# Accustomer/CUDA-AKAZE

Hardware: AMD Instinct MI355X
Metric: pairs_per_sec_detect_describe_match_1080p (higher is better)
Workload: dtype f32; 1 GPU; configs[1]: 1920x1080 grayscale pairs, 4 octaves x 4 sublevels, PM_G2, MLDB-486, max_pts 10000, float path; detect+describe both images + match, D2H included; pairs_per_launch_sequence=256, distinct_pairs_per_gpu=16, float_sequences_enqueued=77, octave_streams=one stream per context, step_pipeline=2, rank0_gpu_numa_node=0

## Files before the change

cuda-akaze_amd/akaze_hip/__init__.py:

```python
import ctypes as C
import os

import numpy as np

try:
    import torch as _torch
except ImportError:
    _torch = None

_HERE = os.path.dirname(os.path.abspath(__file__))
LIB_PATH = os.environ.get("HAK_LIB") or os.path.join(os.path.dirname(_HERE), "libhipakaze.so")

FLEN = 61
MAX_DIST = 96
PM_G1, PM_G2, WEICKERT, CHARBONNIER = 0, 1, 2, 3

POINT_DTYPE = np.dtype([
    ("x", "<f4"), ("y", "<f4"), ("octave", "<i4"), ("response", "<f4"), ("size", "<f4"), ("angle", "<f4"),
    ("features", "u1", (FLEN,)), ("_pad", "u1", (3,)),
    ("match", "<i4"), ("distance", "<i4"), ("match_x", "<f4"), ("match_y", "<f4"),
])
assert POINT_DTYPE.itemsize == 104
MATCH_PAIR_DTYPE = np.dtype([("query", "<i4"), ("train", "<i4"), ("distance", "<i4"), ("second", "<i4"),
                             ("x1", "<f4"), ("y1", "<f4"), ("x2", "<f4"), ("y2", "<f4")])
# ... 100 lines not shown
    "hak_op_hessian": (C.c_int, [_vp, _vp, _vp, _vp, C.c_int, C.c_int, C.c_int, C.c_int]),
    "hak_op_fast_conv_u8": (C.c_int, [_vp, C.c_int, _vp, C.c_int, C.c_int, C.c_int, C.c_float, C.c_int]),
    "hak_op_fast_lowpass": (C.c_int, [_vp, _vp, C.c_int, C.c_int, C.c_int, C.c_float, C.c_int]),
    "hak_op_fast_base": (C.c_int, [_vp, C.c_int, _vp, C.c_int, C.c_int, C.c_int, C.c_float, C.c_int, C.c_float, _ip, _ip, _ip, _ip]),
    "hak_op_fast_down_smooth": (C.c_int, [_vp, _vp, _vp, C.c_int, C.c_int, C.c_int, C.c_int, C.c_int, C.c_int]),
    "hak_op_fast_kcontrast": (C.c_int, [_vp, C.c_int, C.c_int, C.c_int, C.c_float, _ip, _ip, _ip]),
    "hak_op_fast_flow": (C.c_int, [_vp, _vp, C.c_int, C.c_int, C.c_int, C.c_int, C.c_int]),
    "hak_op_fast_smooth_flow": (C.c_int, [_vp, _vp, _vp, C.c_int, C.c_int, C.c_int, C.c_int, C.c_int]),
    "hak_op_fast_nld_steps": (C.c_int, [_vp, _vp, _vp, _vp, C.c_int, C.c_int, C.c_int, _fp, C.c_int]),
    "hak_op_fast_nld_steps_batch": (C.c_int, [_vp, _vp, _vp, _vp, C.c_long, C.c_int, C.c_int, C.c_int, C.c_int, _fp, C.c_int]),
    "hak_op_fast_fed_cycle": (C.c_int, [_vp, C.c_int, C.c_int, C.c_int, C.c_int, _vp, _vp, _vp, _vp, C.c_long, C.c_int, C.c_int, C.c_int,
                                        C.c_int, _ip, _fp, C.c_int]),
    "hak_op_fast_level_tile": (C.c_int, [_vp, C.c_int, C.c_int, C.c_int, C.c_int, _vp, _vp, _vp, C.c_long, C.c_int, C.c_int, C.c_int,
                                         C.c_int, C.c_int, _ip, _fp, C.c_int, _ip]),
    "hak_op_fast_hessian": (C.c_int, [_vp, _vp, _vp, _vp, C.c_int, C.c_int, C.c_int, C.c_int, _ip]),
    "hak_debug_set_plane": (C.c_int, [_vp, C.c_int, C.c_int, C.c_int, C.c_int, _vp]),
    "hak_op_tail_begin": (C.c_int, [_vp]),
    "hak_op_tail_level": (C.c_int, [_vp, C.c_int, C.c_int, _vp]),
    "hak_op_tail_det_level": (C.c_int, [_vp, C.c_int, C.c_int, _vp]),
    "hak_op_tail_seed": (C.c_int, [_vp, _vp, _vp]),
    "hak_debug_tail_total": (C.c_int, [_vp, _ip]),
    "hak_op_fast_tail_level": (C.c_int, [_vp, C.c_int, C.c_int, _vp, C.c_int]),
    "hak_op_fast_tail_det_level": (C.c_int, [_vp, C.c_int, C.c_int, _vp, C.c_int]),
    "hak_debug_tail_maps": (C.c_int, [_vp, _vp, _vp, _vp, C.POINTER(C.c_long), _ip]),
    "hak_op_tail_finish": (C.c_int, [_vp, _vp, C.c_int, C.c_int, C.c_int, _ip]),
    "hak_op_orient_describe": (C.c_int, [_vp, _vp, C.c_int, C.c_int]),
    "hak_op_fast_orient_describe": (C.c_int, [_vp, _vp, C.c_int, C.c_int]),
    "hak_op_copy_probe": (C.c_int, [C.c_long, C.c_int, C.POINTER(C.c_double)]),
    "hak_op_copy_probe_shapes": (C.c_int, [C.c_long, C.c_int, C.POINTER(C.c_double), C.c_int]),
    "hak_op_stream_probe": (C.c_int, [C.c_int, C.c_int, C.c_int, C.c_int, C.c_int, C.c_int, C.POINTER(C.c_double), C.POINTER(C.c_double)]),
# ... 441 lines not shown
```

cuda-akaze_amd/csrc/fed_common.h:

```cpp
#pragma once
#include "hak_internal.h"
#include <type_traits>
#include <utility>

template <typename V> struct FedV;
template <> struct FedV<float> { using V4 = float4; };
template <> struct FedV<int> { using V4 = int4; };
__device__ __forceinline__ float4 mk4(float a, float b, float c, float d) { return make_float4(a, b, c, d); }
__device__ __forceinline__ int4 mk4(int a, int b, int c, int d) { return make_int4(a, b, c, d); }
__device__ __forceinline__ float vadd(float a, float b) { return a + b; }
__device__ __forceinline__ float vsub(float a, float b) { return a - b; }
__device__ __forceinline__ float vmul(float a, float b) { return a * b; }
__device__ __forceinline__ int vadd(int a, int b) { return (int)((unsigned)a + (unsigned)b); }
__device__ __forceinline__ int vsub(int a, int b) { return (int)((unsigned)a - (unsigned)b); }
__device__ __forceinline__ int vmul(int a, int b) { return (int)((unsigned)a * (unsigned)b); }
__device__ __forceinline__ float vstep(float f, float sum, float L) { return fmaf(f, sum, L); }
__device__ __forceinline__ int vstep(int f, int sum, int L) { return vadd(vmul(f, sum >> 16) >> 16, L); }

template <typename V, int NS>
struct FedFacs { V f[NS]; };

__device__ __forceinline__ int hak_dpp_shr1(int v) { return __builtin_amdgcn_update_dpp(0, v, 0x138, 0xf, 0xf, true); }
__device__ __forceinline__ int hak_dpp_shl1(int v) { return __builtin_amdgcn_update_dpp(0, v, 0x130, 0xf, 0xf, true); }
__device__ __forceinline__ float wave_shr1(float v) { return __int_as_float(hak_dpp_shr1(__float_as_int(v))); }
__device__ __forceinline__ float wave_shl1(float v) { return __int_as_float(hak_dpp_shl1(__float_as_int(v))); }
__device__ __forceinline__ int wave_shr1(int v)
{
    int r = hak_dpp_shr1(v);
    asm volatile("" : "+v"(r));
    return r;
}
__device__ __forceinline__ int wave_shl1(int v)
{
    int r = hak_dpp_shl1(v);
    asm volatile("" : "+v"(r));
    return r;
}

typedef float hak_v4f __attribute__((ext_vector_type(4)));
typedef int hak_v4i __attribute__((ext_vector_type(4)));
__device__ __forceinline__ void hak_store_nt(float4* p, const float4 v)
{
    const hak_v4f t = {v.x, v.y, v.z, v.w};
    __builtin_nontemporal_store(t, reinterpret_cast<hak_v4f*>(p));
}
__device__ __forceinline__ void hak_store_nt(int4* p, const int4 v)
{
    const hak_v4i t = {v.x, v.y, v.z, v.w};
    __builtin_nontemporal_store(t, reinterpret_cast<hak_v4i*>(p));
}

typedef unsigned hak_v4u __attribute__((ext_vector_type(4)));
// ... 184 lines not shown
```

cuda-akaze_amd/csrc/hak_test_api.hip:

```cpp
#include "hak_ctx.h"
#include "../../include/hipakaze_test.h"
#include <cmath>
#include <cstdio>
#include <cstring>

extern "C" int hak_debug_plane(hak_ctx* c, int img, int kind, int o, int s, float* h_dst)
{
    if (!c || img < 0 || img >= c->cfg.batch || o < 0 || o >= c->L.noct || s < 0 || s >= c->L.ms) return fail("bad plane");
    const HakLayout& L = c->L;
    const HakOct oc = L.oct[o];
    HIP_TRY(hipStreamSynchronize(c->stream));
    const float* arena = c->arena + (long)img * L.arena;
    if (kind == HAK_PLANE_LT) {
        HIP_TRY(hipMemcpy2D(h_dst, sizeof(float) * oc.w, arena + L.lt(o, s), sizeof(float) * oc.p, sizeof(float) * oc.w, oc.h, hipMemcpyDeviceToHost));
        return 0;
    }
    float* tmp = nullptr;
    HIP_TRY(hipMalloc((void**)&tmp, sizeof(float) * 2 * (size_t)oc.plane));
    int rc = 0;
    const float* src = tmp;
    if (kind == HAK_PLANE_DET) {
        const int step = c->plan[(size_t)o * L.ms + s].sigma_size;
        if (c->last_fast) hakf_launch_det(nullptr, reinterpret_cast<const int*>(arena + L.dxy(o, s)), reinterpret_cast<int*>(tmp), 0, oc.w, oc.h, oc.p, 1, step);
        else hak_launch_hessian(nullptr, arena + L.dxy(o, s), tmp, 0, oc.w, oc.h, oc.p, 1, step);
// ... 393 lines not shown
    const size_t plane = (size_t)h * p;
    int* buf = nullptr;
    HIP_TRY(hipMalloc((void**)&buf, sizeof(int) * 3 * plane));
    int *dxy = buf, *dt = buf + 2 * plane;
    const HakKnobs kn = hak_knobs_from_env();
    const bool fused = hak_launch_hessian_level(nullptr, s, dxy, dt, true, 0, w, h, p, 1, step, nullptr, nullptr, nullptr, 0, 0, 0);
    hak_launch_deinterleave(nullptr, reinterpret_cast<const float*>(dxy), reinterpret_cast<float*>(lx), reinterpret_cast<float*>(ly), w, h, p);
    if (route) *route = !fused ? 3 : (hak_stream_pays(kn.hess_stream, w, h, 1) && hak_hessian_stream_covers(w, h, step, false)) ? 1 : 2;
    int rc = fast_sync("hak_op_fast_hessian");
    if (!rc && fused != (step <= 4)) rc = fail("hak_op_fast_hessian: unexpected route");
    if (!rc && hipMemcpy(det, dt, sizeof(int) * plane, hipMemcpyDeviceToDevice) != hipSuccess) rc = fail("hak_op_fast_hessian: copy");
    (void)hipFree(buf);
    return rc;
}

static HakBatch tail_batch(hak_ctx* c)
{
    HakBatch b{c->arena, c->L.arena, 1, c->state, c->maps, c->L.oct[0].plane, c->bitmap, c->rowcount, c->cand, c->cand_cap, &c->knobs,
               c->perm, c->cfg.max_pts};
    hak_batch_selection(c, b);
    return b;
}
static int tail_level_ok(hak_ctx* c, int o, int s, const void* h)
{
    if (!c || !h) return fail("null argument");
    if (o < 0 || o >= c->L.noct || s < 0 || s >= c->L.ms) return fail("bad level");
    return 0;
}

extern "C" int hak_debug_set_plane(hak_ctx* c, int img, int kind, int o, int s, const float* h_src)
// ... 255 lines not shown
```

cuda-akaze_amd/csrc/kernels_fedsf.hip:

```cpp
#include "fed_common.h"

#ifndef HAK_FS_PD
#define HAK_FS_PD 3
#endif
#ifndef HAK_FS_PD_MAXNS
#define HAK_FS_PD_MAXNS 4
#endif

namespace {

template <typename V, int NS>
struct FsState {
    static constexpr int W = fed_lane_px(NS);
    using Px = FedPx<V, W>;
    static constexpr int GS = fed_gsum_slots(NS);
    static constexpr int UF = fed_unroll(NS);
    static constexpr int PD = NS <= HAK_FS_PD_MAXNS ? HAK_FS_PD : 3;
    Px Lr[6];
    Px Rp[6];
    Px Sm[3];
    V SmL[3], SmR[3];
    Px Lw[NS][2];
    Px Qw[NS][2];
    GHrow<V, W> GH[GS];
// ... 188 lines not shown
        S.GV[i] = zp;
    }
    S.gprev = zp;
#pragma unroll
    for (int i = 0; i < St::PD; i++)
        S.Lq[i] = fs_fetch<DEC, V, W>(L, min(t0 + i, h - 1), lp, xl, sh);
    for (int tb = t0; tb <= tend; tb += UF) {
        if (tb <= NS + 4 || tb + UF - 1 >= h)
            fs_body<V, NS, true, XE, WRITE_G, DEC, WRITE_SM>(std::make_integer_sequence<int, UF>{}, S, tb, L, D, p, xl, x0, w, h, ybeg, yend, owns, fac, kk, ikc, lp, sh, O);
        else
            fs_body<V, NS, false, XE, WRITE_G, DEC, WRITE_SM>(std::make_integer_sequence<int, UF>{}, S, tb, L, D, p, xl, x0, w, h, ybeg, yend, owns, fac, kk, ikc, lp, sh, O);
    }
}

constexpr int fs_hx(int ns) { return ns + 3 <= 8 ? 8 : (ns + 3 + 3) & ~3; }
constexpr int fs_xv(int ns) { return 64 * fed_lane_px(ns) - 2 * fs_hx(ns); }

template <typename V, int NS, bool WRITE_G, bool DEC, bool WRITE_SM>
__global__ __launch_bounds__(256) void k_fed_sf(const V* __restrict__ src, V* __restrict__ smooth, V* __restrict__ flow,
                                                V* __restrict__ dst, long stride, int w, int h, int p,
                                                FedFacs<V, NS> fac, SfTaps<V> kk, const HakImgState* __restrict__ state, int octave,
                                                float fixed_ikc, int ry, int nbx, int nby, int nimg, int lp, int sh)
{
    constexpr int W = fed_lane_px(NS), HX = fs_hx(NS), XV = fs_xv(NS);
    int bx, by, img;
    if (!hak_xcd_decode(nbx, nby, nimg, bx, by, img)) return;
    const V* L = src + (long)img * stride;
    V* SMO = smooth ? smooth + (long)img * stride : nullptr;
    V* GO = flow + (long)img * stride;
    V* D = dst + (long)img * stride;
    const float ikc = state ? state[img].ikc[octave] : fixed_ikc;
    const int lane = threadIdx.x & 63;
    const int wv = __builtin_amdgcn_readfirstlane(threadIdx.x >> 6);
    const int x0 = bx * XV - HX + W * lane;
    const int ybeg = (by * 4 + wv) * ry;
    if (ybeg >= h) return;
    const int yend = min(ybeg + ry, h);
    const bool owns = W * lane >= HX && W * lane < HX + XV && x0 < w && x0 >= 0;
    if (bx == 0 || (bx + 1) * XV + HX >= w) fs_strip<V, NS, true, WRITE_G, DEC, WRITE_SM>(L, SMO, GO, D, w, h, p, fac, kk, ikc, x0, ybeg, yend, owns, lp, sh);
    else fs_strip<V, NS, false, WRITE_G, DEC, WRITE_SM>(L, SMO, GO, D, w, h, p, fac, kk, ikc, x0, ybeg, yend, owns, lp, sh);
}

template <typename V, int NS>
void launch_fs(hipStream_t st, const V* src, V* smooth, V* flow, V* dst, long stride, int w, int h, int p,
               int nimg, SfTaps<V> kk, const float* tau, const HakImgState* state, int octave, float fixed_ikc, bool write_g,
               int sp = 0, int sh = 0)
{
    FedFacs<V, NS> fac;
    for (int k = 0; k < NS; k++) {
        if constexpr (std::is_same<V, float>::value) fac.f[k] = 0.5f * tau[k];
        else fac.f[k] = (int)(0.5f * tau[k] * 65536 + 0.5f);
    }
    constexpr int XV = fs_xv(NS);
    const int gx = (w + XV - 1) / XV;
    const int ry = hak_stream_rows(h, (long)gx * nimg, 8);
    const int gy = (h + 4 * ry - 1) / (4 * ry);
    const unsigned grid = hak_xcd_grid(gx, gy, nimg);
    if (!smooth) {
        if constexpr (std::is_same<V, float>::value) {
            if (write_g) k_fed_sf<V, NS, true, false, false><<<grid, 256, 0, st>>>(src, smooth, flow, dst, stride, w, h, p, fac, kk, state, octave, fixed_ikc, ry, gx, gy, nimg, p, h);
            else k_fed_sf<V, NS, false, false, false><<<grid, 256, 0, st>>>(src, smooth, flow, dst, stride, w, h, p, fac, kk, state, octave, fixed_ikc, ry, gx, gy, nimg, p, h);
        }
    } else if (sp > 0) {
        if (write_g) k_fed_sf<V, NS, true, true, true><<<grid, 256, 0, st>>>(src, smooth, flow, dst, stride, w, h, p, fac, kk, state, octave, fixed_ikc, ry, gx, gy, nimg, sp, sh);
        else k_fed_sf<V, NS, false, true, true><<<grid, 256, 0, st>>>(src, smooth, flow, dst, stride, w, h, p, fac, kk, state, octave, fixed_ikc, ry, gx, gy, nimg, sp, sh);
    } else {
        if (write_g) k_fed_sf<V, NS, true, false, true><<<grid, 256, 0, st>>>(src, smooth, flow, dst, stride, w, h, p, fac, kk, state, octave, fixed_ikc, ry, gx, gy, nimg, p, h);
        else k_fed_sf<V, NS, false, false, true><<<grid, 256, 0, st>>>(src, smooth, flow, dst, stride, w, h, p, fac, kk, state, octave, fixed_ikc, ry, gx, gy, nimg, p, h);
    }
}

template <typename V>
bool launch_fs_any(hipStream_t st, const V* src, V* smooth, V* flow, V* dst, long stride, int w, int h, int p, int nimg,
                   SfTaps<V> kk, int diffusivity, const float* tau, int ns, const HakImgState* state, int octave, float fixed_ikc,
                   bool write_g, int sp = 0, int sh = 0)
{
    constexpr int max_ns = std::is_same<V, float>::value ? HAK_FED_MAX_FUSE : HAK_FED_WIDE_STEPS;
    if (diffusivity != HAK_PM_G2 || (w & 3) || w < 16 || h < 8 || ns < 1 || ns > max_ns) return false;
    if (!smooth && (sp > 0 || !std::is_same<V, float>::value)) return false;
    if ((write_g && smooth ? (flow < smooth ? smooth - flow : flow - smooth) : 0L) + (long)h * p >= (long)HAK_BUF_OOB / (long)sizeof(V)) return false;
    switch (ns) {
    case 1: launch_fs<V, 1>(st, src, smooth, flow, dst, stride, w, h, p, nimg, kk, tau, state, octave, fixed_ikc, write_g, sp, sh); break;
    case 2: launch_fs<V, 2>(st, src, smooth, flow, dst, stride, w, h, p, nimg, kk, tau, state, octave, fixed_ikc, write_g, sp, sh); break;
// ... 64 lines not shown
```

cuda-akaze_amd/csrc/kernels_hessian_stream.hip:

```cpp
#include "fed_common.h"
#include <utility>

namespace {

template <int S, bool LP> struct HsGeo {
    static constexpr int PD = S == 3 ? 1 : 2;
    static constexpr int R = 2 * S + 1 + PD;
    static constexpr int M = LP ? (S <= 2 ? 8 : 12) : (S == 1 ? 4 : S == 4 ? 12 : 8);
    static constexpr int XV = 256 - 2 * M;
    static constexpr int MINW = LP ? (S <= 1 ? 3 : 2) : (S <= 3 ? 3 : 2);
};

template <typename V> struct HsV2;
template <> struct HsV2<float> { using T = float2; };
template <> struct HsV2<int> { using T = int2; };

#define HS_CBUF 256
struct HsCand { unsigned long long* buf; int n; };

template <typename V, int S, bool LP> struct HsState {
    using V4 = typename FedV<V>::V4;
    static constexpr int R = HsGeo<S, LP>::R;
    V4 A[R], X[R];
    V4 W[LP ? R : 1], Rp[LP ? R : 1];
    V4* Y;
    V4* XS;
    V4 Dm, Dc, Dp;
    HsCand cb;
};

template <int I, typename V4> __device__ __forceinline__ auto hs_c(const V4& r)
{
    if constexpr (I == 0) return r.x;
    else if constexpr (I == 1) return r.y;
    else if constexpr (I == 2) return r.z;
    else return r.w;
}
template <int S, int K, typename V4>
__device__ __forceinline__ auto hs_l(const V4& r)
{
    if constexpr (K - S >= 0) return hs_c<K - S>(r);
    else return wave_shr1(hs_c<4 + K - S>(r));
}
template <int S, int K, typename V4>
__device__ __forceinline__ auto hs_r(const V4& r)
{
    if constexpr (K + S <= 3) return hs_c<K + S>(r);
    else return wave_shl1(hs_c<K + S - 4>(r));
}
template <int XE, typename V4>
__device__ __forceinline__ V4 hs_patch(const V4 r, const bool lm1, const bool rp1)
{
    V4 o = r;
    if constexpr ((XE & 1) != 0) {
        const auto c1 = wave_shl1(r.y), c2 = wave_shl1(r.z), c3 = wave_shl1(r.w);
        const auto c4 = wave_shl1(wave_shl1(r.x));
        o.x = lm1 ? c4 : o.x; o.y = lm1 ? c3 : o.y; o.z = lm1 ? c2 : o.z; o.w = lm1 ? c1 : o.w;
    }
    if constexpr ((XE & 2) != 0) {
        const auto m2 = wave_shr1(r.z), m3 = wave_shr1(r.y), m4 = wave_shr1(r.x);
        const auto m5 = wave_shr1(wave_shr1(r.w));
        o.x = rp1 ? m2 : o.x; o.y = rp1 ? m3 : o.y; o.z = rp1 ? m4 : o.z; o.w = rp1 ? m5 : o.w;
    }
// ... 42 lines not shown
{
    const unsigned long long m = __ballot(hit);
    if (m) {
        const int cnt = __popcll(m);
        if (hit) {
            const int fx = x << a.octave, fy = e << a.octave;
            (void)__hip_atomic_fetch_max((hs_gu64p)a.maps + ((long)fy * a.p0 + fx), hak_ext_key(v, a.layer), __ATOMIC_RELAXED,
                                         __HIP_MEMORY_SCOPE_AGENT);
            cb.buf[cb.n + __popcll(m & ((1ull << lane) - 1ull))] = hak_cand_word(a.layer, fx, fy);
        }
        cb.n += cnt;
    }
}

template <typename V, int S, int U, int XE, bool YEDGE, bool LP>
__device__ __forceinline__ void hs_iter(HsState<V, S, LP>& T, const int t, const HsArgs<V>& a, const int xl, const int x0,
                                        const int ybeg, const int yend, const bool owns, const unsigned xok, const int lane,
                                        const __amdgpu_buffer_rsrc_t orsrc, const unsigned (&ovoff)[3], const int er0, const int er1,
                                        const HsCold* cold)
{
    using V4 = typename FedV<V>::V4;
    constexpr int R = HsGeo<S, LP>::R;
    constexpr int PD = HsGeo<S, LP>::PD;
    const V fac1 = a.fac1, fac2 = a.fac2;
    const int w = a.w, h = a.h, p = a.p;
    [[maybe_unused]] const bool le = x0 == 0, re = x0 + 3 == w - 1;
    const bool lm1 = x0 == -4, rp1 = x0 == w;
    if constexpr (!LP) {
        T.A[pmod(U + PD, R)] = hak_load_stream(reinterpret_cast<const V4*>(a.src + (unsigned)(min(t + PD, h - 1) * p + xl)));
    } else {
        const int r = t + 2;
        T.W[pmod(U + 2 + PD, R)] = hak_load_stream(reinterpret_cast<const V4*>(a.src + (unsigned)(min(r + PD, h - 1) * p + xl)));
        const SfTaps<V> kk = a.kk;
        {
            const V4 c = T.W[pmod(U + 2, R)];
            const V sl1 = wave_shr1(c.w), sl2 = wave_shr1(c.z), sr1 = wave_shl1(c.x), sr2 = wave_shl1(c.y);
            V4 l1 = mk4(sl1, c.x, c.y, c.z), l2 = mk4(sl2, sl1, c.x, c.y);
            V4 r1 = mk4(c.y, c.z, c.w, sr1), r2 = mk4(c.z, c.w, sr1, sr2);
            if (XE) {
                l1.x = le ? c.y : l1.x;
                l2.x = le ? c.z : l2.x;
                l2.y = le ? c.y : l2.y;
                r1.w = re ? c.z : r1.w;
                r2.z = re ? c.z : r2.z;
// ... 17 lines not shown
            const V4 u2 = T.Rp[pmod(U - 2, R)], d2 = T.Rp[pmod(U + 2, R)];
            V4 sm;
            sm.x = sf_conv(c.x, u1.x, d1.x, u2.x, d2.x, kk);
            sm.y = sf_conv(c.y, u1.y, d1.y, u2.y, d2.y, kk);
            sm.z = sf_conv(c.z, u1.z, d1.z, u2.z, d2.z, kk);
            sm.w = sf_conv(c.w, u1.w, d1.w, u2.w, d2.w, kk);
            T.A[pmod(U, R)] = sm;
        }
    }
    if constexpr (XE != 0) T.A[pmod(U, R)] = hs_patch<XE>(T.A[pmod(U, R)], lm1, rp1);
    if (YEDGE) {
#pragma unroll
        for (int j = 1; j <= S; j++) {
            if (t == j) T.A[pmod(U - 2 * j, R)] = T.A[pmod(U, R)];
            if (t == h - 1 + j) T.A[pmod(U, R)] = T.A[pmod(U - 2 * j, R)];
        }
    }
    V4 vy_row;
    {
        const int b = t - S;
        const V4 ru = T.A[pmod(U - 2 * S, R)], rc = T.A[pmod(U - S, R)], rl = T.A[pmod(U, R)];
        V4 vx, vy;
#define HS_S1(k, K)                                                                                         \
        {                                                                                                   \
            const V ul = hs_l<S, K>(ru), ur = hs_r<S, K>(ru);                                               \
            const V cl = hs_l<S, K>(rc), cr = hs_r<S, K>(rc);                                               \
            const V ll = hs_l<S, K>(rl), lr = hs_r<S, K>(rl);                                               \
            vx.k = HS_DX(ul, ur, cl, cr, ll, lr);                                                           \
            vy.k = HS_DY(ul, ru.k, ur, ll, rl.k, lr);                                                       \
        }
        HS_S1(x, 0) __builtin_amdgcn_sched_barrier(0); HS_S1(y, 1) __builtin_amdgcn_sched_barrier(0);
        HS_S1(z, 2) __builtin_amdgcn_sched_barrier(0); HS_S1(w, 3) __builtin_amdgcn_sched_barrier(0);
#undef HS_S1
        if constexpr (XE != 0) { vx = hs_patch<XE>(vx, lm1, rp1); vy = hs_patch<XE>(vy, lm1, rp1); }
        T.X[pmod(U, R)] = vx;
        T.Y[pmod(U, R) * 64 + lane] = vy;
        {
            using V2 = typename HsV2<V>::T;
            __builtin_amdgcn_wave_barrier();
            T.XS[lane] = vx;
            __builtin_amdgcn_wave_barrier();
            const V2* xs2 = reinterpret_cast<const V2*>(T.XS);
// ... 66 lines not shown
                hz = hz && hak_ext_strict_max(v.z, up.z, dn.z, v.y, v.w, up.y, up.w, dn.y, dn.w);
                hw = hw && hak_ext_strict_max(v.w, up.w, dn.w, v.z, vr, up.z, ur, dn.z, dr);
                if (T.cb.n > HS_CBUF - 128) hs_flush(T.cb, cold, lane);
                const HsCold ca = *cold;
                hs_emit(hx, v.x, x0, e, ca, lane, T.cb);
                hs_emit(hy, v.y, x0 + 1, e, ca, lane, T.cb);
                hs_emit(hz, v.z, x0 + 2, e, ca, lane, T.cb);
                hs_emit(hw, v.w, x0 + 3, e, ca, lane, T.cb);
            }
        }
    }
}

template <typename V, int S, int XE, bool YEDGE, bool LP, int... U>
__device__ __forceinline__ void hs_group(std::integer_sequence<int, U...>, HsState<V, S, LP>& T, const int tb, const HsArgs<V>& a,
                                         const int xl, const int x0, const int ybeg, const int yend, const bool owns,
                                         const unsigned xok, const int lane, const __amdgpu_buffer_rsrc_t orsrc, const unsigned (&ovoff)[3],
                                         const int er0, const int er1, const HsCold* cold)
{
    (hs_iter<V, S, U, XE, YEDGE, LP>(T, tb + U, a, xl, x0, ybeg, yend, owns, xok, lane, orsrc, ovoff, er0, er1, cold), ...);
}

template <typename V, int S, int XE, bool LP>
__device__ __forceinline__ void hs_strip(const HsArgs<V>& a, const int x0, const int ybeg, const int yend, const bool owns,
                                         const int lane, typename FedV<V>::V4* yring, typename FedV<V>::V4* xstage, unsigned long long* cbuf,
                                         const HsCold* cold)
{
    using G = HsGeo<S, LP>;
    using V4 = typename FedV<V>::V4;
    const int h = a.h, w = a.w;
    const int xl = min(max(x0, 0), a.p - 4);
    const int t0 = LP ? max(max(0, ybeg - 1 - 2 * S) - 4, -2) : max(0, ybeg - 1 - 2 * S);
    const int tend = yend + 2 * S;
    unsigned xok = 0;
#pragma unroll
    for (int k = 0; k < 4; k++)
        if (hak_ext_inside(x0 + k, w, a.ex.psz, a.ex.border)) xok |= 1u << k;
    int er0 = 0, er1 = 0;
    if (a.ex.maps != nullptr) {
        auto row_ok = [&](int e) { return hak_ext_inside(e, h, a.ex.psz, a.ex.border); };
        er0 = ybeg; er1 = yend;
        while (er0 < er1 && !row_ok(er0)) er0++;
        while (er1 > er0 && !row_ok(er1 - 1)) er1--;
    }
    const __amdgpu_buffer_rsrc_t orsrc = hak_buf_rsrc(a.obase);
    const unsigned xb = (unsigned)x0 * (unsigned)sizeof(V);
// ... 10 lines not shown
    T.cb.n = 0;
    const V zz = 0;
    const V4 z4 = mk4(zz, zz, zz, zz);
#pragma unroll
    for (int i = 0; i < G::R; i++) { T.A[i] = T.X[i] = z4; T.Y[i * 64 + lane] = z4; }
    T.Dm = T.Dc = T.Dp = z4;
    if constexpr (LP) {
#pragma unroll
        for (int i = 0; i < G::R; i++) T.W[i] = T.Rp[i] = z4;
#pragma unroll
        for (int i = 0; i < G::PD; i++)
            T.W[pmod(2 + i, G::R)] = hak_load_stream(reinterpret_cast<const V4*>(a.src + (unsigned)(min(t0 + 2 + i, h - 1) * a.p + xl)));
    } else {
#pragma unroll
        for (int i = 0; i < G::PD; i++) T.A[i] = hak_load_stream(reinterpret_cast<const V4*>(a.src + (unsigned)(min(t0 + i, h - 1) * a.p + xl)));
    }
    for (int tb = t0; tb <= tend; tb += G::R) {
        if (tb <= 2 * S || tb + G::R - 1 >= h - (LP ? 2 : 0))
            hs_group<V, S, XE, true, LP>(std::make_integer_sequence<int, G::R>{}, T, tb, a, xl, x0, ybeg, yend, owns, xok, lane, orsrc, ovoff, er0, er1, cold);
        else
            hs_group<V, S, XE, false, LP>(std::make_integer_sequence<int, G::R>{}, T, tb, a, xl, x0, ybeg, yend, owns, xok, lane, orsrc, ovoff, er0, er1, cold);
    }
    if (a.ex.maps != nullptr) hs_flush(T.cb, cold, lane);
}

template <typename V, int S, bool LP>
__global__ __launch_bounds__(256, (HsGeo<S, LP>::MINW)) void k_hessian_stream(HsArgs<V> a, long stride, int ry, int nbx, int nby, int nimg)
{
    using G = HsGeo<S, LP>;
    __shared__ typename FedV<V>::V4 yring[4 * G::R * 64];
    __shared__ typename FedV<V>::V4 xstage[4 * 64];
    __shared__ unsigned long long cbuf[4 * HS_CBUF];
    __shared__ HsCold cold;
    int bx, by, img;
    if (!hak_xcd_decode(nbx, nby, nimg, bx, by, img)) return;
    a.src += (long)img * stride; a.obase += (long)img * stride;
// ... 90 lines not shown
```

cuda-akaze_amd/csrc/kernels_probe.hip:

```cpp
#include "fed_common.h"

template <int NI, bool NT>
__global__ __launch_bounds__(256) void k_copy_probe(const float4* __restrict__ src, float4* __restrict__ dst, long n4)
{
    const long stride = (long)gridDim.x * 256 * NI;
    long i = (long)blockIdx.x * 256 * NI + threadIdx.x;
    for (; i + 256 * (NI - 1) < n4; i += stride) {
        float4 v[NI];
#pragma unroll
        for (int j = 0; j < NI; j++) v[j] = src[i + 256 * j];
#pragma unroll
        for (int j = 0; j < NI; j++) {
            if (NT) hak_store_nt(dst + i + 256 * j, v[j]);
            else dst[i + 256 * j] = v[j];
        }
    }
    for (; i < n4; i += 256) dst[i] = src[i];
}

__global__ __launch_bounds__(256) void k_read_probe(const float4* __restrict__ src, float4* __restrict__ sink, long n4)
{
    const long stride = (long)gridDim.x * 256 * 4;
    float4 acc = make_float4(0.f, 0.f, 0.f, 0.f);
    for (long i = (long)blockIdx.x * 256 * 4 + threadIdx.x; i + 768 < n4; i += stride) {
// ... 57 lines not shown
            const int row = t + u;
            const float4 c = q[u];
            q[u] = hak_load_stream(reinterpret_cast<const float4*>(L + (long)min(row + 3, h - 1) * p + xl));
            acc.x += c.x; acc.y += c.y; acc.z += c.z; acc.w += c.w;
            const unsigned off = (row >= ybeg && row < yend) ? col + (unsigned)row * (unsigned)p * 4u : HAK_BUF_OOB;
#pragma unroll
            for (int k = 0; k < NW; k++) hak_buf_store_nt(r, off + (unsigned)k * (unsigned)(plane * 4), k ? acc : c);
        }
    }
}

template <int S>
__global__ __launch_bounds__(256, (S <= 3 ? 3 : 2)) void k_hess_probe(const float* __restrict__ src, float* __restrict__ dxy, long stride, int w, int h,
                                                                     int p, int ry, int nbx, int nby, int nimg)
{
    constexpr int PD = S == 3 ? 1 : 2, R = 2 * S + 1 + PD, M = S == 1 ? 4 : S == 4 ? 12 : 8, XV = 256 - 2 * M;
    __shared__ float4 yring[4 * R * 64];
    __shared__ float4 xstage[4 * 64];
    __shared__ unsigned long long cbuf[4 * 256];
    int bx, by, img;
    if (!hak_xcd_decode(nbx, nby, nimg, bx, by, img)) return;
    const float* L = src + (long)img * stride;
    float* D = dxy + (long)img * stride * 2;
    const int lane = threadIdx.x & 63;
    const int wv = __builtin_amdgcn_readfirstlane(threadIdx.x >> 6);
    if (threadIdx.x == 0) cbuf[0] = 0;
    const int x0 = bx * XV - M + 4 * lane;
    const int ybeg = (by * 4 + wv) * ry;
    if (ybeg >= h) return;
    const int yend = min(ybeg + ry, h);
    const int xl = min(max(x0, 0), p - 4);
    const int sx = x0 - 4 * lane;
    auto pair_off = [&](int q) -> unsigned {
        const int x = sx + q;
        return q >= M && q < M + XV && x >= 0 && x < w ? (unsigned)x * 8u : HAK_BUF_OOB;
    };
    const unsigned o0 = pair_off(2 * lane), o2 = pair_off(128 + 2 * lane);
    const __amdgpu_buffer_rsrc_t r = hak_buf_rsrc(D);
    float4* Y = yring + wv * R * 64;
    float4* XS = xstage + wv * 64;
    const int t0 = max(0, ybeg - 1 - 2 * S), tend = yend + 2 * S;
    float4 q[PD + 1];
#pragma unroll
    for (int i = 0; i < PD; i++) q[i] = hak_load_stream(reinterpret_cast<const float4*>(L + (unsigned)(min(t0 + i, h - 1) * p + xl)));
    float4 acc = make_float4(0.f, 0.f, 0.f, 0.f);
    int slot = 0;
    for (int t = t0; t <= tend; t += PD + 1) {
#pragma unroll
        for (int u = 0; u <= PD; u++) {
            const int row = t + u;
            q[(u + PD) % (PD + 1)] = hak_load_stream(reinterpret_cast<const float4*>(L + (unsigned)(min(row + PD, h - 1) * p + xl)));
            const float4 c = q[u];
            acc.x += c.x; acc.y += c.y; acc.z += c.z; acc.w += c.w;
            const int b = row - S;
            __builtin_amdgcn_wave_barrier();
            XS[lane] = c;
            Y[slot * 64 + lane] = acc;
            __builtin_amdgcn_wave_barrier();
            const float2* xs2 = reinterpret_cast<const float2*>(XS);
            const float2* ys2 = reinterpret_cast<const float2*>(Y + slot * 64);
            const float2 xa = xs2[lane], ya = ys2[lane], xb = xs2[64 + lane], yb = ys2[64 + lane];
            const unsigned roff = b >= ybeg && b < yend ? (unsigned)(b * p) * 8u : HAK_BUF_OOB;
            hak_buf_store_nt(r, o0 + roff, make_float4(xa.x, ya.x, xa.y, ya.y));
            hak_buf_store_nt(r, o2 + roff, make_float4(xb.x, yb.x, xb.y, yb.y));
            slot = slot + 1 == R ? 0 : slot + 1;
        }
    }
}
// ... 100 lines not shown
    (void)hipEventDestroy(a); (void)hipEventDestroy(b);
    (void)hipFree(s); (void)hipFree(d);
    return rc;
}

int hak_launch_hess_probe(int w, int h, int nimg, int step, int iters, double* ms, double* bytes)
{
    if ((w & 3) || w < 16 || h < 8 || nimg < 1 || step < 1 || step > 4 || iters < 1) return 1;
    const int p = (w + 63) / 64 * 64;
    const long plane = (long)h * p;
    if (2 * plane * 4 >= (long)HAK_BUF_OOB) return 1;
    float *s = nullptr, *d = nullptr;
    if (hipMalloc((void**)&s, sizeof(float) * (size_t)plane * nimg) != hipSuccess) return 1;
    if (hipMalloc((void**)&d, sizeof(float) * (size_t)plane * nimg * 2) != hipSuccess) { (void)hipFree(s); return 1; }
    (void)hipMemset(s, 0, sizeof(float) * (size_t)plane * nimg);
    const int M = step == 1 ? 4 : step == 4 ? 12 : 8, XV = 256 - 2 * M;
    const int gx = (w + XV - 1) / XV;
    const int ry = hak_stream_rows(h, (long)gx * nimg, 16);
    const int gy = (h + 4 * ry - 1) / (4 * ry);
    const unsigned grid = hak_xcd_grid(gx, gy, nimg);
    hipEvent_t a, b;
    (void)hipEventCreate(&a); (void)hipEventCreate(&b);
    auto launch = [&]() {
        switch (step) {
        case 1: k_hess_probe<1><<<grid, 256>>>(s, d, plane, w, h, p, ry, gx, gy, nimg); break;
        case 2: k_hess_probe<2><<<grid, 256>>>(s, d, plane, w, h, p, ry, gx, gy, nimg); break;
        case 3: k_hess_probe<3><<<grid, 256>>>(s, d, plane, w, h, p, ry, gx, gy, nimg); break;
        default: k_hess_probe<4><<<grid, 256>>>(s, d, plane, w, h, p, ry, gx, gy, nimg); break;
        }
    };
    launch();
// ... 10 lines not shown
```

Measured before the change: 6256 pairs/s.

## Shrink halo margins in Hessian stream and FED strip kernels with edge-lane loads

For the non-lowpass step-4 Hessian stream kernel, the x margin drops from 12 to 8 pixels. The two edge lanes that would have needed the wider halo now fetch one extra scalar per row and splice it in through a DPP shift that keeps that value. The FED smooth-flow kernel also picks a smaller halo at runtime when that gives fewer strips for the image width. Both changes aim to cut redundant halo work and strip count, at the cost of an extra scalar load per row, more register state, and a runtime-variable XV. A batched Hessian test entry point and probe updates are added as well.

Result: faster. 6355 pairs/s (median of 6 runs) (+1.6%).

```diff
diff --git a/cuda-akaze_amd/akaze_hip/__init__.py b/cuda-akaze_amd/akaze_hip/__init__.py
--- a/cuda-akaze_amd/akaze_hip/__init__.py
+++ b/cuda-akaze_amd/akaze_hip/__init__.py
@@ -138,6 +138,8 @@
     "hak_op_fast_level_tile": (C.c_int, [_vp, C.c_int, C.c_int, C.c_int, C.c_int, _vp, _vp, _vp, C.c_long, C.c_int, C.c_int, C.c_int,
                                          C.c_int, C.c_int, _ip, _fp, C.c_int, _ip]),
     "hak_op_fast_hessian": (C.c_int, [_vp, _vp, _vp, _vp, C.c_int, C.c_int, C.c_int, C.c_int, _ip]),
+    "hak_op_hessian_batch": (C.c_int, [_vp, _vp, _vp, _vp, C.c_int, C.c_int, C.c_int, C.c_int, C.c_int, _ip]),
+    "hak_op_fast_hessian_batch": (C.c_int, [_vp, _vp, _vp, _vp, C.c_int, C.c_int, C.c_int, C.c_int, C.c_int, _ip]),
     "hak_debug_set_plane": (C.c_int, [_vp, C.c_int, C.c_int, C.c_int, C.c_int, _vp]),
     "hak_op_tail_begin": (C.c_int, [_vp]),
     "hak_op_tail_level": (C.c_int, [_vp, C.c_int, C.c_int, _vp]),
diff --git a/cuda-akaze_amd/csrc/fed_common.h b/cuda-akaze_amd/csrc/fed_common.h
--- a/cuda-akaze_amd/csrc/fed_common.h
+++ b/cuda-akaze_amd/csrc/fed_common.h
@@ -36,6 +36,26 @@
     asm volatile("" : "+v"(r));
     return r;
 }
+__device__ __forceinline__ float wave_shr1_keep(float keep, float v)
+{
+    return __int_as_float(__builtin_amdgcn_update_dpp(__float_as_int(keep), __float_as_int(v), 0x138, 0xf, 0xf, false));
+}
+__device__ __forceinline__ float wave_shl1_keep(float keep, float v)
+{
+    return __int_as_float(__builtin_amdgcn_update_dpp(__float_as_int(keep), __float_as_int(v), 0x130, 0xf, 0xf, false));
+}
+__device__ __forceinline__ int wave_shr1_keep(int keep, int v)
+{
+    int r = __builtin_amdgcn_update_dpp(keep, v, 0x138, 0xf, 0xf, false);
+    asm volatile("" : "+v"(r));
+    return r;
+}
+__device__ __forceinline__ int wave_shl1_keep(int keep, int v)
+{
+    int r = __builtin_amdgcn_update_dpp(keep, v, 0x130, 0xf, 0xf, false);
+    asm volatile("" : "+v"(r));
+    return r;
+}
 
 typedef float hak_v4f __attribute__((ext_vector_type(4)));
 typedef int hak_v4i __attribute__((ext_vector_type(4)));
diff --git a/cuda-akaze_amd/csrc/hak_test_api.hip b/cuda-akaze_amd/csrc/hak_test_api.hip
--- a/cuda-akaze_amd/csrc/hak_test_api.hip
+++ b/cuda-akaze_amd/csrc/hak_test_api.hip
@@ -431,6 +431,38 @@
     return rc;
 }
 
+template <typename V>
+static int hessian_batch_t(const char* who, const V* s, V* lx, V* ly, V* det, int w, int h, int p, int nimg, int step, int* route)
+{
+    if (nimg < 1 || step < 1 || p % 4 || p < w) return fail(std::string(who) + ": nimg < 1, step < 1 or a bad pitch");
+    const size_t plane = (size_t)h * p;
+    const long stride = 4 * (long)plane;
+    V* buf = nullptr;
+    HIP_TRY(hipMalloc((void**)&buf, sizeof(V) * (size_t)stride * nimg));
+    int rc = 0;
+    if (hipMemcpy2D(buf + 3 * plane, sizeof(V) * stride, s, sizeof(V) * plane, sizeof(V) * plane, nimg, hipMemcpyDeviceToDevice) != hipSuccess)
+        rc = fail(std::string(who) + ": copy in");
+    const HakKnobs kn = hak_knobs_from_env();
+    const V thr = 0;
+    if (!rc && !hak_launch_hessian_level(nullptr, buf + 3 * plane, buf, buf + 2 * plane, true, stride, w, h, p, nimg, step, nullptr, nullptr,
+                                         nullptr, 0, 0, thr))
+        rc = fail(std::string(who) + ": the fused kernels do not cover this dilation");
+    for (int i = 0; i < nimg && !rc; i++)
+        hak_launch_deinterleave(nullptr, reinterpret_cast<const float*>(buf + i * stride), reinterpret_cast<float*>(lx + i * plane),
+                                reinterpret_cast<float*>(ly + i * plane), w, h, p);
+    if (route) *route = (hak_stream_pays(kn.hess_stream, w, h, nimg) && hak_hessian_stream_covers(w, h, step, false)) ? 1 : 2;
+    const hipError_t e = hipDeviceSynchronize();
+    if (!rc && e != hipSuccess) rc = fail(std::string(who) + ": " + hipGetErrorString(e));
+    if (!rc && hipMemcpy2D(det, sizeof(V) * plane, buf + 2 * plane, sizeof(V) * stride, sizeof(V) * plane, nimg, hipMemcpyDeviceToDevice) != hipSuccess)
+        rc = fail(std::string(who) + ": copy out");
+    (void)hipFree(buf);
+    return rc;
+}
+extern "C" int hak_op_hessian_batch(const float* s, float* lx, float* ly, float* det, int w, int h, int p, int nimg, int step, int* route)
+{ return hessian_batch_t<float>("hak_op_hessian_batch", s, lx, ly, det, w, h, p, nimg, step, route); }
+extern "C" int hak_op_fast_hessian_batch(const int* s, int* lx, int* ly, int* det, int w, int h, int p, int nimg, int step, int* route)
+{ return hessian_batch_t<int>("hak_op_fast_hessian_batch", s, lx, ly, det, w, h, p, nimg, step, route); }
+
 static HakBatch tail_batch(hak_ctx* c)
 {
     HakBatch b{c->arena, c->L.arena, 1, c->state, c->maps, c->L.oct[0].plane, c->bitmap, c->rowcount, c->cand, c->cand_cap, &c->knobs,
diff --git a/cuda-akaze_amd/csrc/kernels_fedsf.hip b/cuda-akaze_amd/csrc/kernels_fedsf.hip
--- a/cuda-akaze_amd/csrc/kernels_fedsf.hip
+++ b/cuda-akaze_amd/csrc/kernels_fedsf.hip
@@ -226,15 +226,18 @@
 }
 
 constexpr int fs_hx(int ns) { return ns + 3 <= 8 ? 8 : (ns + 3 + 3) & ~3; }
-constexpr int fs_xv(int ns) { return 64 * fed_lane_px(ns) - 2 * fs_hx(ns); }
+constexpr int fs_hx_min(int ns) { return ns + 3 <= 8 ? 8 : (ns + 3 + fed_lane_px(ns) - 1) & ~(fed_lane_px(ns) - 1); }
+static int fs_strips(int ns, int hx, int w) { const int xv = 64 * fed_lane_px(ns) - 2 * hx; return (w + xv - 1) / xv; }
+static int fs_hx_for(int ns, int w) { return fs_strips(ns, fs_hx_min(ns), w) < fs_strips(ns, fs_hx(ns), w) ? fs_hx_min(ns) : fs_hx(ns); }
 
 template <typename V, int NS, bool WRITE_G, bool DEC, bool WRITE_SM>
 __global__ __launch_bounds__(256) void k_fed_sf(const V* __restrict__ src, V* __restrict__ smooth, V* __restrict__ flow,
                                                 V* __restrict__ dst, long stride, int w, int h, int p,
                                                 FedFacs<V, NS> fac, SfTaps<V> kk, const HakImgState* __restrict__ state, int octave,
-                                                float fixed_ikc, int ry, int nbx, int nby, int nimg, int lp, int sh)
-{
-    constexpr int W = fed_lane_px(NS), HX = fs_hx(NS), XV = fs_xv(NS);
+                                                float fixed_ikc, int ry, int nbx, int nby, int nimg, int lp, int sh, int HX)
+{
+    constexpr int W = fed_lane_px(NS);
+    const int XV = 64 * W - 2 * HX;
     int bx, by, img;
     if (!hak_xcd_decode(nbx, nby, nimg, bx, by, img)) return;
     const V* L = src + (long)img * stride;
@@ -263,22 +266,22 @@
         if constexpr (std::is_same<V, float>::value) fac.f[k] = 0.5f * tau[k];
         else fac.f[k] = (int)(0.5f * tau[k] * 65536 + 0.5f);
     }
-    constexpr int XV = fs_xv(NS);
-    const int gx = (w + XV - 1) / XV;
+    const int hx = fs_hx_for(NS, w);
+    const int gx = fs_strips(NS, hx, w);
     const int ry = hak_stream_rows(h, (long)gx * nimg, 8);
     const int gy = (h + 4 * ry - 1) / (4 * ry);
     const unsigned grid = hak_xcd_grid(gx, gy, nimg);
     if (!smooth) {
         if constexpr (std::is_same<V, float>::value) {
-            if (write_g) k_fed_sf<V, NS, true, false, false><<<grid, 256, 0, st>>>(src, smooth, flow, dst, stride, w, h, p, fac, kk, state, octave, fixed_ikc, ry, gx, gy, nimg, p, h);
-            else k_fed_sf<V, NS, false, false, false><<<grid, 256, 0, st>>>(src, smooth, flow, dst, stride, w, h, p, fac, kk, state, octave, fixed_ikc, ry, gx, gy, nimg, p, h);
+            if (write_g) k_fed_sf<V, NS, true, false, false><<<grid, 256, 0, st>>>(src, smooth, flow, dst, stride, w, h, p, fac, kk, state, octave, fixed_ikc, ry, gx, gy, nimg, p, h, hx);
+            else k_fed_sf<V, NS, false, false, false><<<grid, 256, 0, st>>>(src, smooth, flow, dst, stride, w, h, p, fac, kk, state, octave, fixed_ikc, ry, gx, gy, nimg, p, h, hx);
         }
     } else if (sp > 0) {
-        if (write_g) k_fed_sf<V, NS, true, true, true><<<grid, 256, 0, st>>>(src, smooth, flow, dst, stride, w, h, p, fac, kk, state, octave, fixed_ikc, ry, gx, gy, nimg, sp, sh);
-        else k_fed_sf<V, NS, false, true, true><<<grid, 256, 0, st>>>(src, smooth, flow, dst, stride, w, h, p, fac, kk, state, octave, fixed_ikc, ry, gx, gy, nimg, sp, sh);
+        if (write_g) k_fed_sf<V, NS, true, true, true><<<grid, 256, 0, st>>>(src, smooth, flow, dst, stride, w, h, p, fac, kk, state, octave, fixed_ikc, ry, gx, gy, nimg, sp, sh, hx);
+        else k_fed_sf<V, NS, false, true, true><<<grid, 256, 0, st>>>(src, smooth, flow, dst, stride, w, h, p, fac, kk, state, octave, fixed_ikc, ry, gx, gy, nimg, sp, sh, hx);
     } else {
-        if (write_g) k_fed_sf<V, NS, true, false, true><<<grid, 256, 0, st>>>(src, smooth, flow, dst, stride, w, h, p, fac, kk, state, octave, fixed_ikc, ry, gx, gy, nimg, p, h);
-        else k_fed_sf<V, NS, false, false, true><<<grid, 256, 0, st>>>(src, smooth, flow, dst, stride, w, h, p, fac, kk, state, octave, fixed_ikc, ry, gx, gy, nimg, p, h);
+        if (write_g) k_fed_sf<V, NS, true, false, true><<<grid, 256, 0, st>>>(src, smooth, flow, dst, stride, w, h, p, fac, kk, state, octave, fixed_ikc, ry, gx, gy, nimg, p, h, hx);
+        else k_fed_sf<V, NS, false, false, true><<<grid, 256, 0, st>>>(src, smooth, flow, dst, stride, w, h, p, fac, kk, state, octave, fixed_ikc, ry, gx, gy, nimg, p, h, hx);
     }
 }
 
diff --git a/cuda-akaze_amd/csrc/kernels_hessian_stream.hip b/cuda-akaze_amd/csrc/kernels_hessian_stream.hip
--- a/cuda-akaze_amd/csrc/kernels_hessian_stream.hip
+++ b/cuda-akaze_amd/csrc/kernels_hessian_stream.hip
@@ -6,7 +6,8 @@
 template <int S, bool LP> struct HsGeo {
     static constexpr int PD = S == 3 ? 1 : 2;
     static constexpr int R = 2 * S + 1 + PD;
-    static constexpr int M = LP ? (S <= 2 ? 8 : 12) : (S == 1 ? 4 : S == 4 ? 12 : 8);
+    static constexpr int M = LP ? (S <= 2 ? 8 : 12) : (S == 1 ? 4 : 8);
+    static constexpr bool EX = !LP && S == 4;
     static constexpr int XV = 256 - 2 * M;
     static constexpr int MINW = LP ? (S <= 1 ? 3 : 2) : (S <= 3 ? 3 : 2);
 };
@@ -22,6 +23,7 @@
     using V4 = typename FedV<V>::V4;
     static constexpr int R = HsGeo<S, LP>::R;
     V4 A[R], X[R];
+    V E[HsGeo<S, LP>::EX ? R : 1];
     V4 W[LP ? R : 1], Rp[LP ? R : 1];
     V4* Y;
     V4* XS;
@@ -47,6 +49,18 @@
 {
     if constexpr (K + S <= 3) return hs_c<K + S>(r);
     else return wave_shl1(hs_c<K + S - 4>(r));
+}
+template <int S, int K, bool EX, typename V4, typename V>
+__device__ __forceinline__ auto hs_le(const V4& r, const V e)
+{
+    if constexpr (EX && K - S == -1) return wave_shr1_keep(e, r.w);
+    else return hs_l<S, K>(r);
+}
+template <int S, int K, bool EX, typename V4, typename V>
+__device__ __forceinline__ auto hs_re(const V4& r, const V e)
+{
+    if constexpr (EX && K + S == 4) return wave_shl1_keep(e, r.x);
+    else return hs_r<S, K>(r);
 }
 template <int XE, typename V4>
 __device__ __forceinline__ V4 hs_patch(const V4 r, const bool lm1, const bool rp1)
@@ -119,20 +133,22 @@
 }
 
 template <typename V, int S, int U, int XE, bool YEDGE, bool LP>
-__device__ __forceinline__ void hs_iter(HsState<V, S, LP>& T, const int t, const HsArgs<V>& a, const int xl, const int x0,
-                                        const int ybeg, const int yend, const bool owns, const unsigned xok, const int lane,
+__device__ __forceinline__ void hs_iter(HsState<V, S, LP>& T, const int t, const HsArgs<V>& a, const int xl, const int xe,
+                                        const int x0, const int ybeg, const int yend, const bool owns, const unsigned xok, const int lane,
                                         const __amdgpu_buffer_rsrc_t orsrc, const unsigned (&ovoff)[3], const int er0, const int er1,
                                         const HsCold* cold)
 {
     using V4 = typename FedV<V>::V4;
     constexpr int R = HsGeo<S, LP>::R;
     constexpr int PD = HsGeo<S, LP>::PD;
+    constexpr bool EX = HsGeo<S, LP>::EX;
     const V fac1 = a.fac1, fac2 = a.fac2;
     const int w = a.w, h = a.h, p = a.p;
     [[maybe_unused]] const bool le = x0 == 0, re = x0 + 3 == w - 1;
     const bool lm1 = x0 == -4, rp1 = x0 == w;
     if constexpr (!LP) {
         T.A[pmod(U + PD, R)] = hak_load_stream(reinterpret_cast<const V4*>(a.src + (unsigned)(min(t + PD, h - 1) * p + xl)));
+        if constexpr (EX) T.E[pmod(U + PD, R)] = a.src[(unsigned)(min(t + PD, h - 1) * p + xe)];
     } else {
         const int r = t + 2;
         T.W[pmod(U + 2 + PD, R)] = hak_load_stream(reinterpret_cast<const V4*>(a.src + (unsigned)(min(r + PD, h - 1) * p + xl)));
@@ -180,18 +196,25 @@
         for (int j = 1; j <= S; j++) {
             if (t == j) T.A[pmod(U - 2 * j, R)] = T.A[pmod(U, R)];
             if (t == h - 1 + j) T.A[pmod(U, R)] = T.A[pmod(U - 2 * j, R)];
+            if constexpr (EX) {
+                const V en = T.E[pmod(U, R)], eo = T.E[pmod(U - 2 * j, R)];
+                T.E[pmod(U - 2 * j, R)] = t == j ? en : eo;
+                T.E[pmod(U, R)] = t == h - 1 + j ? eo : en;
+            }
         }
     }
     V4 vy_row;
     {
         const int b = t - S;
         const V4 ru = T.A[pmod(U - 2 * S, R)], rc = T.A[pmod(U - S, R)], rl = T.A[pmod(U, R)];
+        V eu = 0, ec = 0, el = 0;
+        if constexpr (EX) { eu = T.E[pmod(U - 2 * S, R)]; ec = T.E[pmod(U - S, R)]; el = T.E[pmod(U, R)]; }
         V4 vx, vy;
 #define HS_S1(k, K)                                                                                         \
         {                                                                                                   \
-            const V ul = hs_l<S, K>(ru), ur = hs_r<S, K>(ru);                                               \
-            const V cl = hs_l<S, K>(rc), cr = hs_r<S, K>(rc);                                               \
-            const V ll = hs_l<S, K>(rl), lr = hs_r<S, K>(rl);                                               \
+            const V ul = hs_le<S, K, EX>(ru, eu), ur = hs_re<S, K, EX>(ru, eu);                             \
+            const V cl = hs_le<S, K, EX>(rc, ec), cr = hs_re<S, K, EX>(rc, ec);                             \
+            const V ll = hs_le<S, K, EX>(rl, el), lr = hs_re<S, K, EX>(rl, el);                             \
             vx.k = HS_DX(ul, ur, cl, cr, ll, lr);                                                           \
             vy.k = HS_DY(ul, ru.k, ur, ll, rl.k, lr);                                                       \
         }
@@ -288,11 +311,11 @@
 
 template <typename V, int S, int XE, bool YEDGE, bool LP, int... U>
 __device__ __forceinline__ void hs_group(std::integer_sequence<int, U...>, HsState<V, S, LP>& T, const int tb, const HsArgs<V>& a,
-                                         const int xl, const int x0, const int ybeg, const int yend, const bool owns,
+                                         const int xl, const int xe, const int x0, const int ybeg, const int yend, const bool owns,
                                          const unsigned xok, const int lane, const __amdgpu_buffer_rsrc_t orsrc, const unsigned (&ovoff)[3],
                                          const int er0, const int er1, const HsCold* cold)
 {
-    (hs_iter<V, S, U, XE, YEDGE, LP>(T, tb + U, a, xl, x0, ybeg, yend, owns, xok, lane, orsrc, ovoff, er0, er1, cold), ...);
+    (hs_iter<V, S, U, XE, YEDGE, LP>(T, tb + U, a, xl, xe, x0, ybeg, yend, owns, xok, lane, orsrc, ovoff, er0, er1, cold), ...);
 }
 
 template <typename V, int S, int XE, bool LP>
@@ -304,6 +327,13 @@
     using V4 = typename FedV<V>::V4;
     const int h = a.h, w = a.w;
     const int xl = min(max(x0, 0), a.p - 4);
+    int xe = 0;
+    if constexpr (G::EX) {
+        const int sx0 = x0 - 4 * lane;
+        xe = lane < 32 ? sx0 - 1 : sx0 + 256;
+        xe = xe >= w ? 2 * (w - 1) - xe : xe;
+        xe = min(max(xe, 0), w - 1);
+    }
     const int t0 = LP ? max(max(0, ybeg - 1 - 2 * S) - 4, -2) : max(0, ybeg - 1 - 2 * S);
     const int tend = yend + 2 * S;
     unsigned xok = 0;
@@ -344,12 +374,18 @@
     } else {
 #pragma unroll
         for (int i = 0; i < G::PD; i++) T.A[i] = hak_load_stream(reinterpret_cast<const V4*>(a.src + (unsigned)(min(t0 + i, h - 1) * a.p + xl)));
+        if constexpr (G::EX) {
+#pragma unroll
+            for (int i = 0; i < G::R; i++) T.E[i] = zz;
+#pragma unroll
+            for (int i = 0; i < G::PD; i++) T.E[i] = a.src[(unsigned)(min(t0 + i, h - 1) * a.p + xe)];
+        }
     }
     for (int tb = t0; tb <= tend; tb += G::R) {
         if (tb <= 2 * S || tb + G::R - 1 >= h - (LP ? 2 : 0))
-            hs_group<V, S, XE, true, LP>(std::make_integer_sequence<int, G::R>{}, T, tb, a, xl, x0, ybeg, yend, owns, xok, lane, orsrc, ovoff, er0, er1, cold);
+            hs_group<V, S, XE, true, LP>(std::make_integer_sequence<int, G::R>{}, T, tb, a, xl, xe, x0, ybeg, yend, owns, xok, lane, orsrc, ovoff, er0, er1, cold);
         else
-            hs_group<V, S, XE, false, LP>(std::make_integer_sequence<int, G::R>{}, T, tb, a, xl, x0, ybeg, yend, owns, xok, lane, orsrc, ovoff, er0, er1, cold);
+            hs_group<V, S, XE, false, LP>(std::make_integer_sequence<int, G::R>{}, T, tb, a, xl, xe, x0, ybeg, yend, owns, xok, lane, orsrc, ovoff, er0, er1, cold);
     }
     if (a.ex.maps != nullptr) hs_flush(T.cb, cold, lane);
 }
diff --git a/cuda-akaze_amd/csrc/kernels_probe.hip b/cuda-akaze_amd/csrc/kernels_probe.hip
--- a/cuda-akaze_amd/csrc/kernels_probe.hip
+++ b/cuda-akaze_amd/csrc/kernels_probe.hip
@@ -95,7 +95,7 @@
 __global__ __launch_bounds__(256, (S <= 3 ? 3 : 2)) void k_hess_probe(const float* __restrict__ src, float* __restrict__ dxy, long stride, int w, int h,
                                                                      int p, int ry, int nbx, int nby, int nimg)
 {
-    constexpr int PD = S == 3 ? 1 : 2, R = 2 * S + 1 + PD, M = S == 1 ? 4 : S == 4 ? 12 : 8, XV = 256 - 2 * M;
+    constexpr int PD = S == 3 ? 1 : 2, R = 2 * S + 1 + PD, M = S == 1 ? 4 : 8, XV = 256 - 2 * M;
     __shared__ float4 yring[4 * R * 64];
     __shared__ float4 xstage[4 * 64];
     __shared__ unsigned long long cbuf[4 * 256];
@@ -112,6 +112,7 @@
     const int yend = min(ybeg + ry, h);
     const int xl = min(max(x0, 0), p - 4);
     const int sx = x0 - 4 * lane;
+    const int xe = min(max(lane < 32 ? sx - 1 : sx + 256, 0), w - 1);
     auto pair_off = [&](int q) -> unsigned {
         const int x = sx + q;
         return q >= M && q < M + XV && x >= 0 && x < w ? (unsigned)x * 8u : HAK_BUF_OOB;
@@ -133,6 +134,7 @@
             q[(u + PD) % (PD + 1)] = hak_load_stream(reinterpret_cast<const float4*>(L + (unsigned)(min(row + PD, h - 1) * p + xl)));
             const float4 c = q[u];
             acc.x += c.x; acc.y += c.y; acc.z += c.z; acc.w += c.w;
+            if constexpr (S == 4) acc.x += L[(unsigned)(min(row + PD, h - 1) * p + xe)];
             const int b = row - S;
             __builtin_amdgcn_wave_barrier();
             XS[lane] = c;
@@ -263,7 +265,7 @@
     if (hipMalloc((void**)&s, sizeof(float) * (size_t)plane * nimg) != hipSuccess) return 1;
     if (hipMalloc((void**)&d, sizeof(float) * (size_t)plane * nimg * 2) != hipSuccess) { (void)hipFree(s); return 1; }
     (void)hipMemset(s, 0, sizeof(float) * (size_t)plane * nimg);
-    const int M = step == 1 ? 4 : step == 4 ? 12 : 8, XV = 256 - 2 * M;
+    const int M = step == 1 ? 4 : 8, XV = 256 - 2 * M;
     const int gx = (w + XV - 1) / XV;
     const int ry = hak_stream_rows(h, (long)gx * nimg, 16);
     const int gy = (h + 4 * ry - 1) / (4 * ry);
```
